# hmc-lair-shark-tracking/auv-sim

Hardware: AMD Instinct MI355X
Metric: RRT-Dubins node expansions/s (RRT.exploring) (higher is better)
Workload: dtype f64; 1 GPU; RRT.exploring 256 obst 200x200 cells 10000 iters x 12288 episodes/GPU, timebin parent sampling; episodes_per_gpu=12288, iters=10000, obstacles=256, cells=40000, parallelism=episodes sharded x1

## Files before the change

auv_sim_amd/_lib.py:

```python
import ctypes as C
import os

import numpy as np

HERE = os.path.dirname(os.path.abspath(__file__))
LIB_PATH = os.environ.get("AUVPLAN_LIBRARY") or os.path.join(HERE, "libauvplan.so")

_dp = C.POINTER(C.c_double)
_ip = C.POINTER(C.c_int32)
_bp = C.POINTER(C.c_int8)


class AuvpError(RuntimeError):
    def __init__(self, code, msg):
        super().__init__("auvplan error %d: %s" % (code, msg))
        self.code = code


class RRTParams(C.Structure):
    _fields_ = [("dist_to_end", C.c_double), ("diff_max", C.c_double), ("freq", C.c_double),
                ("min_dist", C.c_double), ("bin_interval", C.c_double), ("v", C.c_double),
                ("max_traj_time", C.c_double), ("max_plan_time", C.c_double), ("w", C.c_double * 3),
                ("mode", C.c_int32), ("max_iter", C.c_int32), ("points_per_iter", C.c_double)]

# ... 78 lines not shown
    L.auvp_math_dev.argtypes = [vp, C.c_int32, C.c_int32, _dp, _dp, _dp, _dp]
    L.auvp_nn_closest_batch.argtypes = [vp, C.c_int32, _dp, C.c_int32, _dp, C.c_int32, _ip, _ip]
    L.auvp_random_stream_dev.argtypes = [vp, C.c_uint64, C.c_int32, _dp]
    L.auvp_rrt_phase_clocks.argtypes = [vp, C.POINTER(C.c_uint64)]
    L.auvp_last_kernel_ms.argtypes = [vp]
    L.auvp_last_kernel_ms.restype = C.c_double
    L.auvp_last_launch.argtypes = [vp, _ip, _ip, _ip]
    L.auvp_rrt_last_launch_parts.argtypes = [vp, _dp, _dp, _ip]
    L.auvp_rrt_last_leaf_stats.argtypes = [vp, C.POINTER(C.c_int64)]
    L.auvp_rrt_last_kernel.argtypes = [vp]
    L.auvp_rrt_last_kernel.restype = C.c_char_p
    L.auvp_rrt_last_stream_ms.argtypes = [vp]
    L.auvp_rrt_last_stream_ms.restype = C.c_double
    L.auvp_rrt_last_stream_len.argtypes = [vp]
    L.auvp_rrt_last_stream_len.restype = C.c_int64
    L.auvp_hbm_probe.argtypes = [vp, C.c_uint64, C.c_int32, _dp, _dp]
    L.auvp_set_option.argtypes = [vp, C.c_char_p, C.c_int64]
    L.auvp_unset_option.argtypes = [vp, C.c_char_p]
    L.auvp_get_option.argtypes = [vp, C.c_char_p, _ip, C.POINTER(C.c_int64)]
    L.auvp_pipeline_fallbacks.argtypes = [vp, _ip, C.POINTER(C.c_int64)]
    _lib = L
    return L


OPTION_NAMES = ("ROWS", "DUO", "TRIO", "QUAD", "TIGHT_CULL", "NN_EXACT", "LEAF_SWEEP_ALL", "NO_HABITAT_GRID", "RG_MAX_ENTRIES",
                "NO_GRID_INDEX", "PRRT_LAT", "PRRT_PIPE", "PRRT_OBST_LDS", "PRRT_NEXT_LDS", "PRRT_ROWS", "ASTAR_NO_GRID",
                "ASTAR_NO_LIST", "ASTAR_PAIR", "SOG_TILE", "PIPE_FALLBACK", "PRRT_PIPE_DRAW", "PRRT_BUCKET_LDS", "ROWS_STREAM", "ROWS_STREAM_CAP", "ROWS_STREAM_WAVES",
                "ROWS_WG_WAVES")


def _f64(a, shape=None):
    a = np.ascontiguousarray(np.asarray(a, dtype=np.float64))
    return a.reshape(shape) if shape is not None else a


def _p(a, t=_dp):
    return a.ctypes.data_as(t)


def episode_limits(n_episodes, max_traj_time, habitat_keep, n_habitats, mode="timebin", iter_log=False, phase_clocks=False):
    E = int(n_episodes)
    if mode != "timebin":
        raise ValueError("per-episode limits need time-bin mode, not %r" % (mode,))
# ... 2 lines not shown
    mtt = np.broadcast_to(np.asarray(max_traj_time, dtype=np.float64), (E,))
    if not np.all(mtt > 0) or not np.all(np.isfinite(mtt)):
        raise ValueError("every max_traj_time must be finite and > 0")
    allowed = (1 << int(n_habitats)) - 1 if n_habitats < 64 else (1 << 64) - 1
    if habitat_keep is None:
        keep = [allowed] * E
    else:
        keep = [int(k) for k in np.broadcast_to(np.asarray(habitat_keep, dtype=object), (E,))]
    for e, k in enumerate(keep):
        if k < 0 or k & ~allowed:
            raise ValueError("episode %d: habitat_keep 0x%x names habitats outside the table of %d" % (e, k, n_habitats))
    rec = np.zeros(E, dtype=EPISODE_DTYPE)
    rec["max_traj_time"] = mtt
    rec["habitat_keep"] = np.array(keep, dtype=np.uint64)
    return float(mtt.max()), rec


class Context:

    def __init__(self, device=0):
        self.L = load()
        self.h = C.c_void_p()
        rc = self.L.auvp_create(int(device), C.byref(self.h))
        if rc != 0:
            raise AuvpError(rc, "auvp_create(device=%d) failed: no usable HIP device (no CPU fallback)" % device)
        self.device = int(device)
        self.n_episodes = 0
        self.max_iter = 0
        self.world_sizes = {}

# ... 198 lines not shown
        self.L.auvp_prrt_last_kernel.restype = C.c_char_p
        self.L.auvp_prrt_last_kernel.argtypes = [C.c_void_p]
        return (self.L.auvp_prrt_last_kernel(self.h) or b"").decode()

    def last_kernel_ms(self):
        return float(self.L.auvp_last_kernel_ms(self.h))

    def last_launch_parts(self):
        a, b, k = C.c_double(), C.c_double(), C.c_int32()
        self._chk(self.L.auvp_rrt_last_launch_parts(self.h, C.byref(a), C.byref(b), C.byref(k)))
        return a.value, b.value, k.value

    def last_stream_ms(self):
        return float(self.L.auvp_rrt_last_stream_ms(self.h))

    def last_stream_len(self):
        return int(self.L.auvp_rrt_last_stream_len(self.h))

    def last_rrt_kernel(self):
        return (self.L.auvp_rrt_last_kernel(self.h) or b"").decode()

    def last_leaf_stats(self):
        out = (C.c_int64 * 4)()
        self._chk(self.L.auvp_rrt_last_leaf_stats(self.h, out))
        return dict(zip(("nodes_visited", "points_visited", "elements_resummed", "leaves_resummed"), (int(v) for v in out)))

    def hbm_probe(self, n_bytes=4 << 30, reps=3):
        r, c = C.c_double(), C.c_double()
        self._chk(self.L.auvp_hbm_probe(self.h, int(n_bytes), int(reps), C.byref(r), C.byref(c)))
        return r.value, c.value
# ... 6 lines not shown
```

auv_sim_amd/csrc/auvplan.hip:

```cpp
#include <hip/hip_runtime.h>

#include <algorithm>
#include <cmath>
#include <cstdarg>
#include <cstdio>
#include <cstring>
#include <string>
#include <vector>

#include "../../include/auvplan.h"
#include "auvp_seed.h"
#include "rrt_explore_kernel.h"
#include "rrt_rows_kernel.h"
#include "rrt_rows_stream_kernel.h"
#include "rrt_duo_kernel.h"
#include "rrt_trio_kernel.h"

using namespace auvp;

extern "C" hipError_t auvpi_rrt_stream_launch(const auvp::RrtBuffers* B, int n_episodes, hipStream_t stream);
extern "C" hipError_t auvpi_rrt_rows_stream_launch(const auvp::WorldDev* W, const auvp::RrtParamsDev* P, const auvp::RrtBuffers* B, int n_episodes,
                                                   int grid, int block, int lds_max, int lds, hipStream_t stream);
extern "C" hipError_t auvpi_rrt_rows_launch(const auvp::WorldDev* W, const auvp::RrtParamsDev* P, const auvp::RrtBuffers* B, int n_episodes,
                                            int grid, int block, int lds_max, int lds, hipStream_t stream);

static_assert(sizeof(auvp_rrt_summary) == sizeof(RrtSummary), "summary layout");

namespace {

struct DevBuf {
  void* p = nullptr;
  size_t cap = 0;
  ~DevBuf() { if (p) (void)hipFree(p); }
  hipError_t reserve(size_t bytes) {
    if (bytes <= cap) return hipSuccess;
    release();
    hipError_t e = hipMalloc(&p, bytes ? bytes : 16);
    if (e == hipSuccess) cap = bytes ? bytes : 16;
    return e;
  }
  void release() { if (p) { (void)hipFree(p); p = nullptr; cap = 0; } }
  template <class T> T* as() const { return reinterpret_cast<T*>(p); }
};

}

enum AuvpOpt {
  OPT_ROWS, OPT_DUO, OPT_TRIO, OPT_QUAD, OPT_TIGHT_CULL, OPT_NN_EXACT, OPT_LEAF_SWEEP_ALL, OPT_NO_HABITAT_GRID, OPT_RG_MAX_ENTRIES,
  OPT_NO_GRID_INDEX, OPT_PRRT_LAT, OPT_PRRT_PIPE, OPT_PRRT_OBST_LDS, OPT_PRRT_NEXT_LDS, OPT_PRRT_ROWS, OPT_ASTAR_NO_GRID,
  OPT_ASTAR_NO_LIST, OPT_ASTAR_PAIR, OPT_SOG_TILE, OPT_PIPE_FALLBACK, OPT_PRRT_PIPE_DRAW, OPT_PRRT_BUCKET_LDS, OPT_ROWS_STREAM, OPT_ROWS_STREAM_CAP, OPT_ROWS_STREAM_WAVES, OPT_ROWS_WG_WAVES, OPT_COUNT
};
static const char* const AUVP_OPT_NAMES[OPT_COUNT] = {
  "ROWS", "DUO", "TRIO", "QUAD", "TIGHT_CULL", "NN_EXACT", "LEAF_SWEEP_ALL", "NO_HABITAT_GRID", "RG_MAX_ENTRIES",
  "NO_GRID_INDEX", "PRRT_LAT", "PRRT_PIPE", "PRRT_OBST_LDS", "PRRT_NEXT_LDS", "PRRT_ROWS", "ASTAR_NO_GRID",
  "ASTAR_NO_LIST", "ASTAR_PAIR", "SOG_TILE", "PIPE_FALLBACK", "PRRT_PIPE_DRAW", "PRRT_BUCKET_LDS", "ROWS_STREAM", "ROWS_STREAM_CAP", "ROWS_STREAM_WAVES", "ROWS_WG_WAVES"};

struct auvp_handle {
  bool opt_has[OPT_COUNT] = {};
  long long opt_val[OPT_COUNT] = {};
  bool opt_flag(int k, bool dflt) const { return opt_has[k] ? opt_val[k] != 0 : dflt; }
  bool opt_on(int k) const { return opt_has[k] && opt_val[k] != 0; }
  long long opt_num(int k, long long dflt) const { return opt_has[k] ? opt_val[k] : dflt; }
  int device = 0;
  hipStream_t stream = nullptr;
  hipEvent_t ev0 = nullptr, ev1 = nullptr, ev_mid = nullptr, ev_pre = nullptr;
  double last_expand_ms = 0.0, last_leaf_ms = 0.0, last_stream_ms = 0.0;
  long long last_stream_len = 0;
  struct Drawn { RrtParamsDev P{}; long long most = 0; int E = 0; unsigned long long used = 0; bool valid = false; };
  Drawn drawn[4];
  unsigned long long drawn_clock = 0;
  Drawn* drawn_find(const RrtParamsDev& P) {
    for (Drawn& d : drawn)
      if (d.valid && memcmp(&d.P, &P, sizeof P) == 0) return &d;
    return nullptr;
  }
  int last_rows = 0;
  const char* last_rrt_kernel = "";
  std::string err;
  bool have_world = false;
  double obst_area = 0.0;
  WorldDev W{};
  DevBuf d_ox, d_oy, d_ot, d_hab, d_habt, d_poly, d_bins, d_cells, d_prob, d_xoff, d_xitems, d_xdata, d_rgfirst, d_rgbp, d_rgoff,
// ... 763 lines not shown
    hipError_t e = hipFuncSetAttribute(reinterpret_cast<const void*>(kern), hipFuncAttributeMaxDynamicSharedMemorySize, (int)lds);
    if (e != hipSuccess) return e;
    hipLaunchKernelGGL(kern, dim3(grid), dim3(xw * 64), lds, h->stream, h->W, PR, B, (int)E, h->max_pts);
    return hipGetLastError();
  };
  if (B.leaf_stats) HIPCHK(h, hipMemsetAsync(B.leaf_stats, 0, 8 * sizeof(unsigned long long), h->stream));
  HIPCHK(h, hipEventRecord(h->ev0, h->stream));
  hipError_t le = hipSuccess;
  const RowsLdsPlan rp = rrt_rows_lds_plan(P.K, RW_MAX_OBST, rrt_tables_bytes(h->W.n_habitats, h->W.n_poly, h->W.n_bins));
  const bool iter_log = (P.flags & (AUVP_FLAG_ITER_LOG | AUVP_FLAG_PHASE_CLOCKS)) != 0;
  const bool rows_ok = !h->lim && P.mode == 0 && !iter_log && nfreq <= RW_MAX_FREQ && O_ <= RW_MAX_OBST && P.max_iter < 65534 &&
                       rp.total <= 160 * 1024;
  const bool use_rows = rows_ok && h->opt_flag(OPT_ROWS, E > 18 * n_cu_);
  int grid_used = grid, block_used = xw * 64, lds_used = (int)lds;
  bool stream_launched = false;
  const bool duo_ok = !h->lim && P.mode == 0 && !diag && nfreq <= DUO_MAX_FREQ && nfreq >= 1 && O_ <= 256 && h->max_pts <= 64;
  const bool use_duo = duo_ok && !use_rows && !one_wave_only && h->opt_flag(OPT_DUO, E <= 8 * n_cu_);
  const bool use_trio = duo_ok && !use_rows && !one_wave_only && h->opt_flag(OPT_TRIO, E <= TRIO_EP * n_cu_ && !h->opt_on(OPT_DUO));
  h->last_rrt_kernel = use_rows ? "rrt_rows_kernel" : (use_trio ? "rrt_trio_kernel" : (use_duo ? "rrt_duo_kernel" : "rrt_explore_kernel"));
  if (h->lim) h->last_rrt_kernel = "rrt_explore_lim_kernel";
  h->last_stream_ms = 0.0;
  h->last_stream_len = 0;
  if (use_trio) {
    int eps_wg = (E + n_cu_ - 1) / n_cu_;
    eps_wg = eps_wg < 1 ? 1 : (eps_wg > TRIO_EP ? TRIO_EP : eps_wg);
    const int jd = O_ <= 64 ? 1 : (O_ <= 128 ? 2 : 4);
    const int dl = trio_lds_bytes(P.K, jd * 64, rrt_tables_bytes(h->W.n_habitats, h->W.n_poly, h->W.n_bins), eps_wg);
    if (dl > 160 * 1024) return fail(h, AUVP_ERR_ARG, "LDS need %d B > 160 KiB (K=%d)", dl, P.K);
    const bool quad = h->opt_flag(OPT_QUAD, E <= n_cu_);
    grid_used = (E + eps_wg - 1) / eps_wg; block_used = eps_wg * (quad ? 256 : 192); lds_used = dl;
// ... 38 lines not shown
      cap = rrt_stream_len(h, seen);
      if (cap > 0x7fffffffll) use_stream = false;
      else if (!rrt_stream_reserve(h, (size_t)E * (size_t)cap * sizeof(double), &grew)) {
        if (h->opt_on(OPT_ROWS_STREAM)) return fail(h, AUVP_ERR_CAPACITY, "ROWS_STREAM = 1: %zu bytes of random stream do not fit the free memory", (size_t)E * (size_t)cap * sizeof(double));
        use_stream = false;
      }
    }
    if (grew) HIPCHK(h, hipEventRecord(h->ev0, h->stream));
    if (use_stream) {
      RrtBuffers Bs = B;
      Bs.stream = h->d_stream.as<double>();
      Bs.stream_cap = cap;
      int sw = (int)h->opt_num(OPT_ROWS_WG_WAVES, (E + RW_ROWS * n_cu - 1) / (RW_ROWS * n_cu));
      const int sw_max = (int)h->opt_num(OPT_ROWS_STREAM_WAVES, RW_WAVES);
      sw = sw < 1 ? 1 : (sw > sw_max ? sw_max : sw);
      sw = sw > RW_WAVES ? RW_WAVES : sw;
      while (sw > 1 && rrt_rows_stream_lds_plan(P.K, RW_MAX_OBST, rrt_tables_bytes(h->W.n_habitats, h->W.n_poly, h->W.n_bins), sw).total > 160 * 1024) sw--;
      const RowsStreamLdsPlan sp = rrt_rows_stream_lds_plan(P.K, RW_MAX_OBST, rrt_tables_bytes(h->W.n_habitats, h->W.n_poly, h->W.n_bins), sw);
      const RowsStreamLdsPlan sp_max = sp;
      grid_used = (E + sw * RW_ROWS - 1) / (sw * RW_ROWS); block_used = sw * 64;
      lds_used = sp.total;
      h->last_rrt_kernel = "rrt_rows_stream_kernel";
      h->last_stream_len = cap;
      le = auvpi_rrt_stream_launch(&Bs, (int)E, h->stream);
      if (le == hipSuccess) le = hipEventRecord(h->ev_pre, h->stream);
      if (le == hipSuccess) le = auvpi_rrt_rows_stream_launch(&h->W, &PR, &Bs, (int)E, grid_used, block_used, sp_max.total, sp.total, h->stream);
      stream_launched = true;
    } else
    le = auvpi_rrt_rows_launch(&h->W, &PR, &B, (int)E, grid_used, block_used, rp.total, rq.total, h->stream);
  } else {
  const int jsel = O <= 64 ? 0 : (O <= 128 ? 1 : (O <= 256 ? 2 : (O <= 512 ? 3 : 4)));
  const RrtEpisodeLimDev* lim = h->d_lim.as<RrtEpisodeLimDev>();
  auto launch_lim = [&](auto kern) -> hipError_t {
    hipError_t e = hipFuncSetAttribute(reinterpret_cast<const void*>(kern), hipFuncAttributeMaxDynamicSharedMemorySize, (int)lds);
    if (e != hipSuccess) return e;
    hipLaunchKernelGGL(kern, dim3(grid), dim3(xw * 64), lds, h->stream, h->W, PR, B, (int)E, h->max_pts, lim);
    return hipGetLastError();
  };
#define AUVP_LAUNCH_J(JV)                                                                   \
  do {                                                                                      \
    if (h->lim) le = launch_lim(rrt_explore_lim_kernel<JV>);                                \
// ... 226 lines not shown
double auvp_last_kernel_ms(auvp_handle* h) { return h ? h->last_ms : -1.0; }

int auvp_rrt_last_launch_parts(auvp_handle* h, double* expand_ms, double* leaf_ms, int32_t* episodes_per_wave) {
  if (!h) return AUVP_ERR_ARG;
  if (!h->have_batch) return fail(h, AUVP_ERR_STATE, "no batch has run");
  if (expand_ms) *expand_ms = h->last_expand_ms;
  if (leaf_ms) *leaf_ms = h->last_leaf_ms;
  if (episodes_per_wave) *episodes_per_wave = h->last_rows ? 4 : 1;
  return AUVP_OK;
}

const char* auvp_rrt_last_kernel(auvp_handle* h) { return h ? h->last_rrt_kernel : ""; }

double auvp_rrt_last_stream_ms(auvp_handle* h) { return h ? h->last_stream_ms : -1.0; }
int64_t auvp_rrt_last_stream_len(auvp_handle* h) { return h ? (int64_t)h->last_stream_len : -1; }

int auvp_rrt_last_leaf_stats(auvp_handle* h, int64_t* out4) {
  if (!h || !out4) return AUVP_ERR_ARG;
  if (!h->have_batch || !h->B.leaf_stats) return fail(h, AUVP_ERR_STATE, "no batch has run");
  HIPCHK(h, hipSetDevice(h->device));
  HIPCHK(h, hipMemcpy(out4, h->B.leaf_stats, 4 * sizeof(int64_t), hipMemcpyDeviceToHost));
  return AUVP_OK;
}

int auvp_last_launch(auvp_handle* h, int32_t* grid, int32_t* block, int32_t* lds_bytes) {
  if (!h) return AUVP_ERR_ARG;
  if (grid) *grid = h->last_grid;
  if (block) *block = h->last_block;
  if (lds_bytes) *lds_bytes = h->last_lds;
  return AUVP_OK;
// ... 29 lines not shown
```

auv_sim_amd/csrc/rows_kernels.hip:

```cpp
#include <hip/hip_runtime.h>
#include <stdint.h>

#include "rrt_rows_kernel.h"
#include "rrt_rows_stream_kernel.h"
#include "rrt_stream_kernel.h"

extern "C" __attribute__((visibility("hidden"))) hipError_t auvpi_rrt_rows_launch(const auvp::WorldDev* W, const auvp::RrtParamsDev* P,
                                                                                  const auvp::RrtBuffers* B, int n_episodes, int grid,
                                                                                  int block, int lds_max, int lds, hipStream_t stream) {
  hipError_t e = hipFuncSetAttribute(reinterpret_cast<const void*>(auvp::rrt_rows_kernel), hipFuncAttributeMaxDynamicSharedMemorySize, lds_max);
  if (e != hipSuccess) return e;
  hipLaunchKernelGGL(auvp::rrt_rows_kernel, dim3(grid), dim3(block), lds, stream, *W, *P, *B, n_episodes);
  return hipGetLastError();
}

extern "C" __attribute__((visibility("hidden"))) hipError_t auvpi_rrt_stream_launch(const auvp::RrtBuffers* B, int n_episodes, hipStream_t stream) {
  const int grid = (n_episodes + auvp::RSTREAM_WAVES - 1) / auvp::RSTREAM_WAVES;
  hipLaunchKernelGGL(auvp::rrt_stream_kernel, dim3(grid), dim3(auvp::RSTREAM_WAVES * 64), 0, stream, *B, n_episodes);
  return hipGetLastError();
}
extern "C" __attribute__((visibility("hidden"))) hipError_t auvpi_rrt_rows_stream_launch(const auvp::WorldDev* W, const auvp::RrtParamsDev* P,
                                                                                         const auvp::RrtBuffers* B, int n_episodes, int grid,
                                                                                         int block, int lds_max, int lds, hipStream_t stream) {
  auto go = [&](auto kern) -> hipError_t {
    hipError_t e = hipFuncSetAttribute(reinterpret_cast<const void*>(kern), hipFuncAttributeMaxDynamicSharedMemorySize, lds_max);
    if (e != hipSuccess) return e;
    hipLaunchKernelGGL(kern, dim3(grid), dim3(block), lds, stream, *W, *P, *B, n_episodes);
    return hipGetLastError();
  };
  return go(auvp::rrt_rows_stream_kernel<auvp::RW_WAVES>);
}
```

auv_sim_amd/csrc/rrt_rows_body.h:

```cpp
  extern __shared__ __align__(16) unsigned char smem[];
  const RrtTables S = rrt_tables_view(smem, W.n_habitats, W.n_poly);
  const int wave = (int)(threadIdx.x >> 6);
  const int lane = lane_id();
  const int row = lane >> 4, rl = lane & 15, rowbase = lane & 48;
  const int K = P.K;
  const int wg_waves = (int)(blockDim.x >> 6);
#if AUVP_ROWS_BODY_STREAM
  const RowsStreamLdsPlan plan = rrt_rows_stream_lds_plan(K, RW_MAX_OBST, rrt_tables_bytes(W.n_habitats, W.n_poly, W.n_bins), wg_waves);
  unsigned char* ebase = smem + plan.tables + (size_t)(wave * RW_ROWS + row) * plan.per_ep;
  double* ring = reinterpret_cast<double*>(ebase);
  double* inc = reinterpret_cast<double*>(ebase + plan.ring);
  uint16_t* bin_count = reinterpret_cast<uint16_t*>(ebase + plan.ring + plan.scratch);
#else
  const RowsLdsPlan plan = rrt_rows_lds_plan(K, RW_MAX_OBST, rrt_tables_bytes(W.n_habitats, W.n_poly, W.n_bins), wg_waves);
  unsigned char* ebase = smem + plan.tables + (size_t)(wave * RW_ROWS + row) * plan.per_ep;
  uint32_t* mt = reinterpret_cast<uint32_t*>(ebase);
  double* win = reinterpret_cast<double*>(ebase + plan.mt);
  double* inc = win;
  uint16_t* bin_count = reinterpret_cast<uint16_t*>(ebase + plan.mt + plan.scratch);
#endif

  rrt_tables_stage(S, W);
  if (threadIdx.x == 0) *S.params = P;
  const RrtParamsDev& Q = *S.params;
// ... 12 lines not shown
  double* nodeF = B.node_f + (size_t)eps * capn * 8;
  int4* nodeI = reinterpret_cast<int4*>(B.node_i) + (size_t)eps * capn;
  uint8_t* nodeQ = B.node_q + (size_t)eps * capn;
  double* ptF = B.points + (size_t)eps * capp * 6;
  const BinLists bins = bin_lists(B, (size_t)eps, K);
  int next_chunk = 0;
  const double* init = B.init + (size_t)eps * 6;

#if AUVP_ROWS_BODY_STREAM
  RowStream rng;
  rng.ring = ring;
  rng.src = B.stream + (size_t)eps * (size_t)B.stream_cap;
  rng.pos = 0u; rng.front = 0u; rng.req = 0u;
  rng.cap = (uint32_t)B.stream_cap;
#pragma unroll
  for (int c = 0; c < RS_PEND; c++) rng.pend[c] = 0.0;
#define ROWS_CONSUME(on, n) stream_advance(rng, on, (uint32_t)(n))
#else
  RowRng rng;
  rng.s = mt;
  for (int i = rl; i < 624; i += 16) mt[i] = B.mt[(size_t)eps * 624 + i];
  {
    int idx = B.mt_index ? B.mt_index[eps] : 624;
    idx = idx < 0 ? 0 : (idx > 624 ? 624 : idx);
    rng.pslot = idx == 624 ? 0u : (uint32_t)idx;
    rng.avail = (uint32_t)(624 - idx);
    rng.drawn = 0ull;
  }
#define ROWS_CONSUME(on, n) rows_advance(rng, on, (uint32_t)(2 * (n)))
#endif
  for (int i = rl; i < K + 2; i += 16) bin_count[i] = 0;
// ... 5 lines not shown
    bins.direct[(K >= 1 ? 1 : 0) * AUVP_BIN_HEAD] = 0;
    bin_count[K >= 1 ? 1 : 0] = 1;
  }
  wave_sync();
  int n_nodes = 1, n_points = 0, status = 0, n_cand = 0, iters_run = 0;
  const double4 sbox = reinterpret_cast<const double4*>(W.os_box)[rl];
  const int nv_poly = W.n_poly;

  for (int it = 0; it < P.max_iter; it++) {
    if (!wave_any(live)) break;
    int par = 0, n_total = 0, base = 0;
    {
      bool search = live;
      int fo = 0, rb = 0, cnt = 0;
      double u = 0.0;
      for (;;) {
#if AUVP_ROWS_BODY_STREAM
        if (!stream_ensure(rng, search, 16u, rl) && search) { status = AUVP_ST_STREAM; live = false; iters_run = it; search = false; }
        if (search) u = stream_at(rng, (uint32_t)rl);
#else
        rows_ensure(rng, search, 32u, rl);
        if (search) { u = rows_random_at(rng, (uint32_t)rl); win[rl] = u; }
#endif
        const int rbj = (int)py_uniform(1.0, (double)(K + 1), u);
        const bool cand = search && rl < 14;
        const bool badkey = cand && rbj > K;
        const int cj = (cand && !badkey) ? (int)bin_count[rbj] : 0;
        const uint32_t okm = row_ballot(cj != 0, rowbase), badm = row_ballot(badkey, rowbase);
        const int f_ok = okm ? (__ffs((int)okm) - 1) : 16, f_bad = badm ? (__ffs((int)badm) - 1) : 16;
        if (search) {
          if (f_bad < f_ok) { status = -5; live = false; iters_run = it; search = false; }
          else if (f_ok < 16) { fo = f_ok; search = false; }
        }
        const bool again = search;
        ROWS_CONSUME(again, 14);
        const int src = rowbase + (again ? 0 : fo);
        const int rb_n = row_read(rbj, src), cnt_n = row_read(cj, src);
        if (!again && live && cnt == 0) { rb = rb_n; cnt = cnt_n; }
        if (!wave_any(again)) break;
      }
#if AUVP_ROWS_BODY_STREAM
      const double u1 = stream_at(rng, (uint32_t)(fo + 1)), u2 = stream_at(rng, (uint32_t)(fo + 2));
#else
      wave_sync();
      const double u1 = win[fo + 1], u2 = win[fo + 2];
#endif
      if (live) {
        const int ri = (int)py_uniform(0.0, (double)cnt, u1);
        par = bin_member(bins, rb, ri);
        n_total = (int)auvp_floor(py_uniform(0.0, Q.freq, u2) / 1);
        base = fo + 3;
      }
    }
    const bool on0 = live && 0 < n_total;
    const int n0_ = on0 ? (n_total < RW_C ? n_total : RW_C) : 0;
#if AUVP_ROWS_BODY_STREAM
    if (!stream_ensure(rng, on0, (uint32_t)(base + 3 * n0_), rl) && on0) { status = AUVP_ST_STREAM; live = false; iters_run = it; }
#else
    auto make_window = [&](bool on, int nwin, int b0) {
      rows_ensure(rng, on, (uint32_t)(2 * (b0 + nwin)), rl);
#pragma unroll
      for (int t = 0; t < 3; t++) {
        const int j = rl + 16 * t;
        if (on && j < nwin) win[j] = rows_random_at(rng, (uint32_t)(b0 + j));
      }
      wave_sync();
    };
    {
      const int e_end = base + 3 * n0_;
      rows_ensure(rng, on0, (uint32_t)(2 * e_end), rl);
#pragma unroll
      for (int t = 0; t < 3; t++) {
        const int e = 16 + rl + 16 * t;
        if (on0 && e < e_end) win[e] = rows_random_at(rng, (uint32_t)e);
      }
      wave_sync();
    }
#endif
    double cx = 0.0, cy = 0.0, cth = 0.0, ctt = 0.0, clen = 0.0;
    if (live) {
      const double2 a = *reinterpret_cast<const double2*>(nodeF + (size_t)par * 8);
      const double2 b = *reinterpret_cast<const double2*>(nodeF + (size_t)par * 8 + 2);
      cx = a.x; cy = a.y; cth = b.x; ctt = b.y;
      clen = nodeF[(size_t)par * 8 + 4];
    }
#if AUVP_ROWS_BODY_STREAM
    stream_top_up(rng, live, rl);
#endif
    const double px0 = cx, py0 = cy, clen0 = clen;
    int cnt = 0;
    double ptx[2] = {0.0, 0.0}, pty[2] = {0.0, 0.0};
    bool ptv[2] = {false, false};
    bool first_pass = true;
#pragma unroll
    for (int pass = 0; pass < 2; pass++) {
      const int c0 = pass * RW_C;
      const bool on = live && c0 < n_total;
      if (!wave_any(on)) break;
      const int n = on ? ((n_total - c0) < RW_C ? (n_total - c0) : RW_C) : 0;
      const int nwin = 3 * n;
#ifdef AUVP_ROWS_PAD
      {
        double pd0 = cth, pd1 = cx, pd2 = cy, pd3 = ctt;
#pragma unroll
        for (int q = 0; q < AUVP_ROWS_PAD / 4; q++)
          asm volatile("v_add_f64 %0, %0, 1.0\n\tv_add_f64 %1, %1, 1.0\n\tv_add_f64 %2, %2, 1.0\n\tv_add_f64 %3, %3, 1.0"
                       : "+v"(pd0), "+v"(pd1), "+v"(pd2), "+v"(pd3));
      }
#endif
      const int b0 = first_pass ? base : 0;
#if AUVP_ROWS_BODY_STREAM
      if (pass != 0 && !stream_ensure(rng, on, (uint32_t)nwin, rl) && on) { status = AUVP_ST_STREAM; live = false; iters_run = it; }
      const uint32_t wb = (uint32_t)b0;
#define ROWS_WIN(j) stream_at(rng, wb + (uint32_t)(j))
#else
      if (pass != 0) make_window(on, nwin, b0);
      const double* wp = win + (pass == 0 ? base : 0);
#define ROWS_WIN(j) wp[j]
#endif
      unsigned long long tpred = 0ull;
#pragma unroll
      for (int t = 0; t < 3; t++) {
        const int j = rl + 16 * t;
        const double dist = py_uniform(0.0, Q.dist_to_end, ROWS_WIN(j));
        const double diff = py_uniform(-Q.diff_max, Q.diff_max, ROWS_WIN(j + 1));
        const unsigned long long fb = __builtin_amdgcn_fcmp(auvp_fabs(dist), auvp_fabs(diff), 2 ) &
                                      __builtin_amdgcn_uicmp((unsigned)(j + 1), (unsigned)nwin, 36 );
        tpred |= ((fb >> rowbase) & 0xffffull) << (16 * t);
      }
// ... 198 lines not shown
          nf[4] = clen;
          nodeI[me] = make_int4(it, par, n_points, cnt);
          nodeQ[me] = ctt >= Q.max_traj_time - 30 ? 1 : 0;
        }
        n_nodes++;
        n_points += cnt;
      }
    }
    wave_sync();
  }

  const bool valid = ep < n_episodes;
  if (live) iters_run = P.max_iter;
#if AUVP_ROWS_BODY_STREAM
  const unsigned long long drawn = 2ull * rng.pos;
  if (!stream_ensure(rng, valid && status == 0, 1u, rl) && valid && status == 0) status = AUVP_ST_STREAM;
  const double after = status == AUVP_ST_STREAM ? 0.0 : stream_at(rng, 0u);
#else
  const unsigned long long drawn = rng.drawn;
  rows_ensure(rng, valid, 2u, rl);
  const double after = rows_random_at(rng, 0u);
#endif
  if (valid) {
    for (int i = rl; i < K + 1; i += 16) B.bin_count[(size_t)ep * (K + 1) + i] = (int32_t)bin_count[i];
    if (rl == 0) {
      RrtSummary& s = B.summary[ep];
#if AUVP_ROWS_BODY_STREAM
      pipe_report(B.pipe_fail, status == AUVP_ST_STREAM ? AUVP_ST_PIPELINE : 0);
#endif
      s.status = status; s.n_nodes = n_nodes; s.n_points = n_points; s.n_leaves = 0;
      s.best_leaf = -1; s.best_path_len = 0; s.iters_run = iters_run; s.n_candidates = n_cand;
      s.best_cost[0] = __builtin_inf(); s.best_cost[1] = 0.0; s.best_cost[2] = 0.0; s.best_cost[3] = 0.0;
      s.best_length = 0.0;
      s.rng_after = after; s.leaf_elems = 0; s.n_draw32 = drawn; s.nn_scanned = 0ull;
    }
  }
#undef ROWS_CONSUME
```

auv_sim_amd/csrc/rrt_rows_stream_kernel.h:

```cpp
#ifndef AUVP_RRT_ROWS_STREAM_KERNEL_H
#define AUVP_RRT_ROWS_STREAM_KERNEL_H
#include "rrt_rows_kernel.h"

namespace auvp {

constexpr int RS_RING = 256;
constexpr int RS_WAVES = 16;
constexpr int RS_PEND = 4;

struct RowsStreamLdsPlan {
  int tables, ring, scratch, bins, per_ep, obst, total;
};
__host__ __device__ inline RowsStreamLdsPlan rrt_rows_stream_lds_plan(int K, int n_obst_slots, int tables_bytes, int waves = RW_WAVES) {
  RowsStreamLdsPlan p;
  p.tables = (tables_bytes + 15) & ~15;
  p.ring = RS_RING * 8;
  p.scratch = (4 * 18 * 8 + 15) & ~15;
  p.bins = (((K + 2) * 2) + 15) & ~15;
  p.per_ep = p.ring + p.scratch + p.bins;
  p.obst = n_obst_slots * (8 + 8 + 4);
  p.total = p.tables + waves * RW_ROWS * p.per_ep + p.obst;
  return p;
}

struct RowStream {
  double* ring;
  const double* src;
  uint32_t pos, front, req, cap;
  double pend[RS_PEND];
};

__device__ __forceinline__ void stream_commit(RowStream& r, int rl) {
#pragma unroll
  for (int c = 0; c < RS_PEND; c++)
    if (r.front + 16u * (uint32_t)c < r.req) r.ring[(r.front + 16u * (uint32_t)c + (uint32_t)rl) & (uint32_t)(RS_RING - 1)] = r.pend[c];
  r.front = r.req;
}
__device__ __forceinline__ void stream_request(RowStream& r, bool on, int rl) {
  const uint32_t room = (uint32_t)RS_RING - (r.front - r.pos);
  uint32_t n = room >> 4;
  n = n > (uint32_t)RS_PEND ? (uint32_t)RS_PEND : n;
  n = on ? n : 0u;
#pragma unroll
  for (int c = 0; c < RS_PEND; c++) {
    const uint32_t e = r.req + 16u * (uint32_t)c + (uint32_t)rl;
    if ((uint32_t)c < n && e < r.cap) r.pend[c] = __builtin_nontemporal_load(r.src + e);
  }
  r.req += 16u * n;
}
__device__ __forceinline__ void stream_top_up(RowStream& r, bool on, int rl) {
  stream_commit(r, rl);
  stream_request(r, on, rl);
}
__device__ __forceinline__ bool stream_ensure(RowStream& r, bool want, uint32_t need, int rl) {
  const uint32_t need_w = want ? need : 0u;
  const bool ok = r.pos + need_w <= r.cap;
  for (;;) {
    if (__builtin_amdgcn_uicmp(r.front - r.pos, ok ? need_w : 0u, 36 ) == 0ull) break;
    const bool go = ok && r.front - r.pos < need_w;
    stream_commit(r, rl);
    stream_request(r, go && ok, rl);
    stream_commit(r, rl);
    wave_sync();
    if (!wave_any(go && ok && r.front - r.pos < need_w)) break;
  }
  wave_sync();
  return ok;
}
__device__ __forceinline__ double stream_at(const RowStream& r, uint32_t j) { return r.ring[(r.pos + j) & (uint32_t)(RS_RING - 1)]; }
__device__ __forceinline__ void stream_advance(RowStream& r, bool on, uint32_t n) {
  if (on) r.pos += n;
}

template <int MAXW>
static __global__ __launch_bounds__(MAXW * 64, 1) void rrt_rows_stream_kernel(WorldDev W, RrtParamsDev P, RrtBuffers B, int n_episodes) {
#define AUVP_ROWS_BODY_STREAM 1
#include "rrt_rows_body.h"
#undef AUVP_ROWS_BODY_STREAM
}

}
#endif
```

include/auvplan.h:

```cpp
#ifndef AUVPLAN_H
#define AUVPLAN_H
#include <stdint.h>

#ifdef __cplusplus
extern "C" {
#endif

typedef struct auvp_handle auvp_handle;

enum {
  AUVP_OK = 0,
  AUVP_NO_QUALIFYING_LEAF = 1,
  AUVP_ERR_ARG = -1,
  AUVP_ERR_CAPACITY = -2,
  AUVP_ERR_HIP = -3,
  AUVP_ERR_STATE = -4,
  AUVP_ERR_KEY = -5,
  AUVP_ERR_COMM = -6,
  AUVP_ERR_GENERATOR = -7,
  AUVP_ERR_PIPELINE = -9
  ,
  AUVP_ERR_STREAM = -10
};

// ... 167 lines not shown
int auvp_cost_paths(auvp_handle* h, int32_t n_paths, const int32_t* off, const double* pts_xyt,
                    const int32_t* bin_lo, const int32_t* bin_hi, const double* total_traj_time,
                    const double* weights3, double* out4);
int auvp_nn_closest_batch(auvp_handle* h, int32_t n_nodes, const double* xy, int32_t n_queries, const double* q,
                          int32_t force_exact, int32_t* out_index, int32_t* out_slow);
int auvp_hbm_probe(auvp_handle* h, uint64_t bytes, int32_t reps, double* read_GBps, double* copy_GBps);
int auvp_sincos_dev(auvp_handle* h, int32_t n, const double* x, double* s, double* c);
int auvp_math_dev(auvp_handle* h, int32_t op, int32_t n, const double* a, const double* b, double* out0, double* out1);
int auvp_random_stream_dev(auvp_handle* h, uint64_t seed, int32_t n, double* out);

int auvp_rrt_phase_clocks(auvp_handle* h, uint64_t* out);
double auvp_last_kernel_ms(auvp_handle* h);
int auvp_rrt_last_launch_parts(auvp_handle* h, double* expand_ms, double* leaf_ms, int32_t* episodes_per_wave);
double auvp_rrt_last_stream_ms(auvp_handle* h);
int64_t auvp_rrt_last_stream_len(auvp_handle* h);
const char* auvp_rrt_last_kernel(auvp_handle* h);
int auvp_rrt_last_leaf_stats(auvp_handle* h, int64_t* out4);
int auvp_last_launch(auvp_handle* h, int32_t* grid, int32_t* block, int32_t* lds_bytes);

int auvp_prrt_replan_particles(auvp_handle* h, const double* start4, const auvp_prrt_params* params, const double* xform,
                               const double* clamp4, uint64_t seed_base, int32_t flags);

#define AUVP_COMM_ID_BYTES 128
int auvp_comm_unique_id(uint8_t* id_out );
int auvp_comm_init(auvp_handle* h, int32_t world_size, int32_t rank, const uint8_t* id);
int auvp_comm_destroy(auvp_handle* h);
int auvp_gather(auvp_handle* h, const void* send_dev, size_t bytes_per_rank, void* recv_dev);
int auvp_gather_var(auvp_handle* h, const void* send_dev, int64_t send_bytes, void* recv_dev, int64_t recv_cap_bytes,
                    int64_t* counts_out);
int auvp_gather_counts(auvp_handle* h, int64_t send_bytes, int64_t* counts_out );
// ... 17 lines not shown
```

Before: 1.262 billion expansions/s.

## Add mirrored LDS ring tail and vectorized f64x2 stream loads for rows-stream RRT

The random-number ring in LDS gains a mirrored tail of 48 extra slots, so window reads can use a plain base-plus-offset address without masking on every access. Global stream loads and LDS commits now move two doubles per lane as an f64x2 vector, with fewer pending chunks. A shape planner picks waves per workgroup and whether the mirror fits the LDS budget, and can drop waves to make it fit. The costs are extra LDS per episode, which may reduce waves per workgroup, and a new requirement that the stream capacity is a multiple of 64.

```diff
diff --git a/auv_sim_amd/_lib.py b/auv_sim_amd/_lib.py
--- a/auv_sim_amd/_lib.py
+++ b/auv_sim_amd/_lib.py
@@ -116,6 +116,9 @@
     L.auvp_rrt_last_stream_ms.restype = C.c_double
     L.auvp_rrt_last_stream_len.argtypes = [vp]
     L.auvp_rrt_last_stream_len.restype = C.c_int64
+    if hasattr(L, "auvp_rrt_last_stream_mirror"):
+        L.auvp_rrt_last_stream_mirror.argtypes = [vp]
+        L.auvp_rrt_rows_stream_shape.argtypes = [C.c_int32] * 6 + [_ip, _ip, _ip]
     L.auvp_hbm_probe.argtypes = [vp, C.c_uint64, C.c_int32, _dp, _dp]
     L.auvp_set_option.argtypes = [vp, C.c_char_p, C.c_int64]
     L.auvp_unset_option.argtypes = [vp, C.c_char_p]
@@ -128,7 +131,7 @@
 OPTION_NAMES = ("ROWS", "DUO", "TRIO", "QUAD", "TIGHT_CULL", "NN_EXACT", "LEAF_SWEEP_ALL", "NO_HABITAT_GRID", "RG_MAX_ENTRIES",
                 "NO_GRID_INDEX", "PRRT_LAT", "PRRT_PIPE", "PRRT_OBST_LDS", "PRRT_NEXT_LDS", "PRRT_ROWS", "ASTAR_NO_GRID",
                 "ASTAR_NO_LIST", "ASTAR_PAIR", "SOG_TILE", "PIPE_FALLBACK", "PRRT_PIPE_DRAW", "PRRT_BUCKET_LDS", "ROWS_STREAM", "ROWS_STREAM_CAP", "ROWS_STREAM_WAVES",
-                "ROWS_WG_WAVES")
+                "ROWS_WG_WAVES", "ROWS_STREAM_MIRROR")
 
 
 def _f64(a, shape=None):
@@ -161,6 +164,15 @@
     rec["max_traj_time"] = mtt
     rec["habitat_keep"] = np.array(keep, dtype=np.uint64)
     return float(mtt.max()), rec
+
+
+def rows_stream_shape(K, n_habitats, n_poly, n_bins, waves_wanted=12, force=-1):
+    w, m, l = C.c_int32(), C.c_int32(), C.c_int32()
+    rc = load().auvp_rrt_rows_stream_shape(int(K), int(n_habitats), int(n_poly), int(n_bins), int(waves_wanted), int(force),
+                                           C.byref(w), C.byref(m), C.byref(l))
+    if rc != 0:
+        raise AuvpError(rc, "auvp_rrt_rows_stream_shape: bad argument")
+    return w.value, bool(m.value), l.value
 
 
 class Context:
@@ -389,6 +401,9 @@
     def last_stream_ms(self):
         return float(self.L.auvp_rrt_last_stream_ms(self.h))
 
+    def last_stream_mirror(self):
+        return int(self.L.auvp_rrt_last_stream_mirror(self.h))
+
     def last_stream_len(self):
         return int(self.L.auvp_rrt_last_stream_len(self.h))
 
diff --git a/auv_sim_amd/csrc/auvplan.hip b/auv_sim_amd/csrc/auvplan.hip
--- a/auv_sim_amd/csrc/auvplan.hip
+++ b/auv_sim_amd/csrc/auvplan.hip
@@ -20,7 +20,7 @@
 
 extern "C" hipError_t auvpi_rrt_stream_launch(const auvp::RrtBuffers* B, int n_episodes, hipStream_t stream);
 extern "C" hipError_t auvpi_rrt_rows_stream_launch(const auvp::WorldDev* W, const auvp::RrtParamsDev* P, const auvp::RrtBuffers* B, int n_episodes,
-                                                   int grid, int block, int lds_max, int lds, hipStream_t stream);
+                                                   int grid, int block, int lds_max, int lds, int mirror, hipStream_t stream);
 extern "C" hipError_t auvpi_rrt_rows_launch(const auvp::WorldDev* W, const auvp::RrtParamsDev* P, const auvp::RrtBuffers* B, int n_episodes,
                                             int grid, int block, int lds_max, int lds, hipStream_t stream);
 
@@ -48,12 +48,12 @@
 enum AuvpOpt {
   OPT_ROWS, OPT_DUO, OPT_TRIO, OPT_QUAD, OPT_TIGHT_CULL, OPT_NN_EXACT, OPT_LEAF_SWEEP_ALL, OPT_NO_HABITAT_GRID, OPT_RG_MAX_ENTRIES,
   OPT_NO_GRID_INDEX, OPT_PRRT_LAT, OPT_PRRT_PIPE, OPT_PRRT_OBST_LDS, OPT_PRRT_NEXT_LDS, OPT_PRRT_ROWS, OPT_ASTAR_NO_GRID,
-  OPT_ASTAR_NO_LIST, OPT_ASTAR_PAIR, OPT_SOG_TILE, OPT_PIPE_FALLBACK, OPT_PRRT_PIPE_DRAW, OPT_PRRT_BUCKET_LDS, OPT_ROWS_STREAM, OPT_ROWS_STREAM_CAP, OPT_ROWS_STREAM_WAVES, OPT_ROWS_WG_WAVES, OPT_COUNT
+  OPT_ASTAR_NO_LIST, OPT_ASTAR_PAIR, OPT_SOG_TILE, OPT_PIPE_FALLBACK, OPT_PRRT_PIPE_DRAW, OPT_PRRT_BUCKET_LDS, OPT_ROWS_STREAM, OPT_ROWS_STREAM_CAP, OPT_ROWS_STREAM_WAVES, OPT_ROWS_WG_WAVES, OPT_ROWS_STREAM_MIRROR, OPT_COUNT
 };
 static const char* const AUVP_OPT_NAMES[OPT_COUNT] = {
   "ROWS", "DUO", "TRIO", "QUAD", "TIGHT_CULL", "NN_EXACT", "LEAF_SWEEP_ALL", "NO_HABITAT_GRID", "RG_MAX_ENTRIES",
   "NO_GRID_INDEX", "PRRT_LAT", "PRRT_PIPE", "PRRT_OBST_LDS", "PRRT_NEXT_LDS", "PRRT_ROWS", "ASTAR_NO_GRID",
-  "ASTAR_NO_LIST", "ASTAR_PAIR", "SOG_TILE", "PIPE_FALLBACK", "PRRT_PIPE_DRAW", "PRRT_BUCKET_LDS", "ROWS_STREAM", "ROWS_STREAM_CAP", "ROWS_STREAM_WAVES", "ROWS_WG_WAVES"};
+  "ASTAR_NO_LIST", "ASTAR_PAIR", "SOG_TILE", "PIPE_FALLBACK", "PRRT_PIPE_DRAW", "PRRT_BUCKET_LDS", "ROWS_STREAM", "ROWS_STREAM_CAP", "ROWS_STREAM_WAVES", "ROWS_WG_WAVES", "ROWS_STREAM_MIRROR"};
 
 struct auvp_handle {
   bool opt_has[OPT_COUNT] = {};
@@ -66,6 +66,7 @@
   hipEvent_t ev0 = nullptr, ev1 = nullptr, ev_mid = nullptr, ev_pre = nullptr;
   double last_expand_ms = 0.0, last_leaf_ms = 0.0, last_stream_ms = 0.0;
   long long last_stream_len = 0;
+  int last_stream_mirror = -1;
   struct Drawn { RrtParamsDev P{}; long long most = 0; int E = 0; unsigned long long used = 0; bool valid = false; };
   Drawn drawn[4];
   unsigned long long drawn_clock = 0;
@@ -859,6 +860,7 @@
   const bool use_rows = rows_ok && h->opt_flag(OPT_ROWS, E > 18 * n_cu_);
   int grid_used = grid, block_used = xw * 64, lds_used = (int)lds;
   bool stream_launched = false;
+  h->last_stream_mirror = -1;
   const bool duo_ok = !h->lim && P.mode == 0 && !diag && nfreq <= DUO_MAX_FREQ && nfreq >= 1 && O_ <= 256 && h->max_pts <= 64;
   const bool use_duo = duo_ok && !use_rows && !one_wave_only && h->opt_flag(OPT_DUO, E <= 8 * n_cu_);
   const bool use_trio = duo_ok && !use_rows && !one_wave_only && h->opt_flag(OPT_TRIO, E <= TRIO_EP * n_cu_ && !h->opt_on(OPT_DUO));
@@ -927,17 +929,19 @@
       int sw = (int)h->opt_num(OPT_ROWS_WG_WAVES, (E + RW_ROWS * n_cu - 1) / (RW_ROWS * n_cu));
       const int sw_max = (int)h->opt_num(OPT_ROWS_STREAM_WAVES, RW_WAVES);
       sw = sw < 1 ? 1 : (sw > sw_max ? sw_max : sw);
-      sw = sw > RW_WAVES ? RW_WAVES : sw;
-      while (sw > 1 && rrt_rows_stream_lds_plan(P.K, RW_MAX_OBST, rrt_tables_bytes(h->W.n_habitats, h->W.n_poly, h->W.n_bins), sw).total > 160 * 1024) sw--;
-      const RowsStreamLdsPlan sp = rrt_rows_stream_lds_plan(P.K, RW_MAX_OBST, rrt_tables_bytes(h->W.n_habitats, h->W.n_poly, h->W.n_bins), sw);
+      const RowsStreamShape shape = rrt_rows_stream_shape(P.K, RW_MAX_OBST, rrt_tables_bytes(h->W.n_habitats, h->W.n_poly, h->W.n_bins), sw,
+                                                          h->opt_has[OPT_ROWS_STREAM_MIRROR] ? (h->opt_val[OPT_ROWS_STREAM_MIRROR] != 0 ? 1 : 0) : -1);
+      sw = shape.waves;
+      const RowsStreamLdsPlan sp = shape.plan;
       const RowsStreamLdsPlan sp_max = sp;
+      h->last_stream_mirror = shape.mirror ? 1 : 0;
       grid_used = (E + sw * RW_ROWS - 1) / (sw * RW_ROWS); block_used = sw * 64;
       lds_used = sp.total;
       h->last_rrt_kernel = "rrt_rows_stream_kernel";
       h->last_stream_len = cap;
       le = auvpi_rrt_stream_launch(&Bs, (int)E, h->stream);
       if (le == hipSuccess) le = hipEventRecord(h->ev_pre, h->stream);
-      if (le == hipSuccess) le = auvpi_rrt_rows_stream_launch(&h->W, &PR, &Bs, (int)E, grid_used, block_used, sp_max.total, sp.total, h->stream);
+      if (le == hipSuccess) le = auvpi_rrt_rows_stream_launch(&h->W, &PR, &Bs, (int)E, grid_used, block_used, sp_max.total, sp.total, shape.mirror ? 1 : 0, h->stream);
       stream_launched = true;
     } else
     le = auvpi_rrt_rows_launch(&h->W, &PR, &B, (int)E, grid_used, block_used, rp.total, rq.total, h->stream);
@@ -1194,6 +1198,17 @@
 
 double auvp_rrt_last_stream_ms(auvp_handle* h) { return h ? h->last_stream_ms : -1.0; }
 int64_t auvp_rrt_last_stream_len(auvp_handle* h) { return h ? (int64_t)h->last_stream_len : -1; }
+int auvp_rrt_last_stream_mirror(auvp_handle* h) { return h ? h->last_stream_mirror : -1; }
+
+int auvp_rrt_rows_stream_shape(int32_t K, int32_t n_habitats, int32_t n_poly, int32_t n_bins, int32_t waves_wanted, int32_t force,
+                               int32_t* waves, int32_t* mirror, int32_t* lds_bytes) {
+  if (K < 0 || n_habitats < 0 || n_poly < 0 || n_bins < 0) return AUVP_ERR_ARG;
+  const RowsStreamShape s = rrt_rows_stream_shape(K, RW_MAX_OBST, rrt_tables_bytes(n_habitats, n_poly, n_bins), waves_wanted, force);
+  if (waves) *waves = s.waves;
+  if (mirror) *mirror = s.mirror ? 1 : 0;
+  if (lds_bytes) *lds_bytes = s.plan.total;
+  return AUVP_OK;
+}
 
 int auvp_rrt_last_leaf_stats(auvp_handle* h, int64_t* out4) {
   if (!h || !out4) return AUVP_ERR_ARG;
diff --git a/auv_sim_amd/csrc/rows_kernels.hip b/auv_sim_amd/csrc/rows_kernels.hip
--- a/auv_sim_amd/csrc/rows_kernels.hip
+++ b/auv_sim_amd/csrc/rows_kernels.hip
@@ -21,12 +21,13 @@
 }
 extern "C" __attribute__((visibility("hidden"))) hipError_t auvpi_rrt_rows_stream_launch(const auvp::WorldDev* W, const auvp::RrtParamsDev* P,
                                                                                          const auvp::RrtBuffers* B, int n_episodes, int grid,
-                                                                                         int block, int lds_max, int lds, hipStream_t stream) {
+                                                                                         int block, int lds_max, int lds, int mirror, hipStream_t stream) {
+  if (B->stream_cap <= 0 || B->stream_cap % 64 != 0) return hipErrorInvalidValue;
   auto go = [&](auto kern) -> hipError_t {
     hipError_t e = hipFuncSetAttribute(reinterpret_cast<const void*>(kern), hipFuncAttributeMaxDynamicSharedMemorySize, lds_max);
     if (e != hipSuccess) return e;
     hipLaunchKernelGGL(kern, dim3(grid), dim3(block), lds, stream, *W, *P, *B, n_episodes);
     return hipGetLastError();
   };
-  return go(auvp::rrt_rows_stream_kernel<auvp::RW_WAVES>);
+  return mirror ? go(auvp::rrt_rows_stream_kernel<auvp::RW_WAVES>) : go(auvp::rrt_rows_stream_masked_kernel<auvp::RW_WAVES>);
 }
diff --git a/auv_sim_amd/csrc/rrt_rows_body.h b/auv_sim_amd/csrc/rrt_rows_body.h
--- a/auv_sim_amd/csrc/rrt_rows_body.h
+++ b/auv_sim_amd/csrc/rrt_rows_body.h
@@ -6,7 +6,7 @@
   const int K = P.K;
   const int wg_waves = (int)(blockDim.x >> 6);
 #if AUVP_ROWS_BODY_STREAM
-  const RowsStreamLdsPlan plan = rrt_rows_stream_lds_plan(K, RW_MAX_OBST, rrt_tables_bytes(W.n_habitats, W.n_poly, W.n_bins), wg_waves);
+  const RowsStreamLdsPlan plan = rrt_rows_stream_lds_plan(K, RW_MAX_OBST, rrt_tables_bytes(W.n_habitats, W.n_poly, W.n_bins), wg_waves, MIRROR);
   unsigned char* ebase = smem + plan.tables + (size_t)(wave * RW_ROWS + row) * plan.per_ep;
   double* ring = reinterpret_cast<double*>(ebase);
   double* inc = reinterpret_cast<double*>(ebase + plan.ring);
@@ -50,7 +50,10 @@
   rng.pos = 0u; rng.front = 0u; rng.req = 0u;
   rng.cap = (uint32_t)B.stream_cap;
 #pragma unroll
-  for (int c = 0; c < RS_PEND; c++) rng.pend[c] = 0.0;
+  for (int c = 0; c < RS_PEND; c++) rng.pend[c] = rs_piece(0.0);
+#ifdef AUVP_STREAM_COUNT_SLOW
+  rng.slow = 0u;
+#endif
 #define ROWS_CONSUME(on, n) stream_advance(rng, on, (uint32_t)(n))
 #else
   RowRng rng;
@@ -86,10 +89,14 @@
       bool search = live;
       int fo = 0, rb = 0, cnt = 0;
       double u = 0.0;
+#if AUVP_ROWS_BODY_STREAM
+      StreamBase<MIRROR> sel;
+#endif
       for (;;) {
 #if AUVP_ROWS_BODY_STREAM
-        if (!stream_ensure(rng, search, 16u, rl) && search) { status = AUVP_ST_STREAM; live = false; iters_run = it; search = false; }
-        if (search) u = stream_at(rng, (uint32_t)rl);
+        if (!stream_ensure<MIRROR>(rng, search, 16u, rl) && search) { status = AUVP_ST_STREAM; live = false; iters_run = it; search = false; }
+        sel = stream_base<MIRROR>(rng, 0u, rl);
+        if (search) u = stream_read(sel, rl, rl);
 #else
         rows_ensure(rng, search, 32u, rl);
         if (search) { u = rows_random_at(rng, (uint32_t)rl); win[rl] = u; }
@@ -112,7 +119,7 @@
         if (!wave_any(again)) break;
       }
 #if AUVP_ROWS_BODY_STREAM
-      const double u1 = stream_at(rng, (uint32_t)(fo + 1)), u2 = stream_at(rng, (uint32_t)(fo + 2));
+      const double u1 = stream_read(sel, fo + 1, rl), u2 = stream_read(sel, fo + 2, rl);
 #else
       wave_sync();
       const double u1 = win[fo + 1], u2 = win[fo + 2];
@@ -127,7 +134,7 @@
     const bool on0 = live && 0 < n_total;
     const int n0_ = on0 ? (n_total < RW_C ? n_total : RW_C) : 0;
 #if AUVP_ROWS_BODY_STREAM
-    if (!stream_ensure(rng, on0, (uint32_t)(base + 3 * n0_), rl) && on0) { status = AUVP_ST_STREAM; live = false; iters_run = it; }
+    if (!stream_ensure<MIRROR>(rng, on0, (uint32_t)(base + 3 * n0_), rl) && on0) { status = AUVP_ST_STREAM; live = false; iters_run = it; }
 #else
     auto make_window = [&](bool on, int nwin, int b0) {
       rows_ensure(rng, on, (uint32_t)(2 * (b0 + nwin)), rl);
@@ -157,7 +164,7 @@
       clen = nodeF[(size_t)par * 8 + 4];
     }
 #if AUVP_ROWS_BODY_STREAM
-    stream_top_up(rng, live, rl);
+    stream_top_up<MIRROR>(rng, live, rl);
 #endif
     const double px0 = cx, py0 = cy, clen0 = clen;
     int cnt = 0;
@@ -182,9 +189,9 @@
 #endif
       const int b0 = first_pass ? base : 0;
 #if AUVP_ROWS_BODY_STREAM
-      if (pass != 0 && !stream_ensure(rng, on, (uint32_t)nwin, rl) && on) { status = AUVP_ST_STREAM; live = false; iters_run = it; }
-      const uint32_t wb = (uint32_t)b0;
-#define ROWS_WIN(j) stream_at(rng, wb + (uint32_t)(j))
+      if (pass != 0 && !stream_ensure<MIRROR>(rng, on, (uint32_t)nwin, rl) && on) { status = AUVP_ST_STREAM; live = false; iters_run = it; }
+      const StreamBase<MIRROR> wb = stream_base<MIRROR>(rng, (uint32_t)b0, rl);
+#define ROWS_WIN(j) stream_read(wb, (j), rl)
 #else
       if (pass != 0) make_window(on, nwin, b0);
       const double* wp = win + (pass == 0 ? base : 0);
@@ -413,8 +420,8 @@
   if (live) iters_run = P.max_iter;
 #if AUVP_ROWS_BODY_STREAM
   const unsigned long long drawn = 2ull * rng.pos;
-  if (!stream_ensure(rng, valid && status == 0, 1u, rl) && valid && status == 0) status = AUVP_ST_STREAM;
-  const double after = status == AUVP_ST_STREAM ? 0.0 : stream_at(rng, 0u);
+  if (!stream_ensure<MIRROR>(rng, valid && status == 0, 1u, rl) && valid && status == 0) status = AUVP_ST_STREAM;
+  const double after = status == AUVP_ST_STREAM ? 0.0 : stream_read(stream_base<MIRROR>(rng, 0u, rl), rl, rl);
 #else
   const unsigned long long drawn = rng.drawn;
   rows_ensure(rng, valid, 2u, rl);
@@ -432,6 +439,9 @@
       s.best_cost[0] = __builtin_inf(); s.best_cost[1] = 0.0; s.best_cost[2] = 0.0; s.best_cost[3] = 0.0;
       s.best_length = 0.0;
       s.rng_after = after; s.leaf_elems = 0; s.n_draw32 = drawn; s.nn_scanned = 0ull;
+#if AUVP_ROWS_BODY_STREAM && defined(AUVP_STREAM_COUNT_SLOW)
+      s.nn_scanned = rng.slow;
+#endif
     }
   }
 #undef ROWS_CONSUME
diff --git a/auv_sim_amd/csrc/rrt_rows_stream_kernel.h b/auv_sim_amd/csrc/rrt_rows_stream_kernel.h
--- a/auv_sim_amd/csrc/rrt_rows_stream_kernel.h
+++ b/auv_sim_amd/csrc/rrt_rows_stream_kernel.h
@@ -5,16 +5,27 @@
 namespace auvp {
 
 constexpr int RS_RING = 256;
+constexpr int RS_MIRROR = 48;
 constexpr int RS_WAVES = 16;
-constexpr int RS_PEND = 4;
+#ifndef AUVP_RS_PIECE
+#define AUVP_RS_PIECE 2
+#endif
+constexpr int RS_PIECE = AUVP_RS_PIECE;
+constexpr int RS_CHUNK = 16 * RS_PIECE;
+constexpr int RS_PEND = 64 / RS_CHUNK;
+typedef double rs_f64x2 __attribute__((ext_vector_type(2)));
+template <int N> struct RsPiece { typedef double type; };
+template <> struct RsPiece<2> { typedef rs_f64x2 type; };
+typedef RsPiece<RS_PIECE>::type rs_piece;
+constexpr int RS_LDS_LIMIT = 160 * 1024;
 
 struct RowsStreamLdsPlan {
   int tables, ring, scratch, bins, per_ep, obst, total;
 };
-__host__ __device__ inline RowsStreamLdsPlan rrt_rows_stream_lds_plan(int K, int n_obst_slots, int tables_bytes, int waves = RW_WAVES) {
+__host__ __device__ inline RowsStreamLdsPlan rrt_rows_stream_lds_plan(int K, int n_obst_slots, int tables_bytes, int waves = RW_WAVES, bool mirror = false) {
   RowsStreamLdsPlan p;
   p.tables = (tables_bytes + 15) & ~15;
-  p.ring = RS_RING * 8;
+  p.ring = (RS_RING + (mirror ? RS_MIRROR : 0)) * 8;
   p.scratch = (4 * 18 * 8 + 15) & ~15;
   p.bins = (((K + 2) * 2) + 15) & ~15;
   p.per_ep = p.ring + p.scratch + p.bins;
@@ -23,57 +34,102 @@
   return p;
 }
 
+struct RowsStreamShape {
+  int waves;
+  bool mirror;
+  RowsStreamLdsPlan plan;
+};
+__host__ inline RowsStreamShape rrt_rows_stream_shape(int K, int n_obst_slots, int tables_bytes, int waves_wanted, int force = -1) {
+  int sw = waves_wanted < 1 ? 1 : (waves_wanted > RW_WAVES ? RW_WAVES : waves_wanted);
+  while (sw > 1 && rrt_rows_stream_lds_plan(K, n_obst_slots, tables_bytes, sw, false).total > RS_LDS_LIMIT) sw--;
+  bool mirror = force < 0 ? rrt_rows_stream_lds_plan(K, n_obst_slots, tables_bytes, sw, true).total <= RS_LDS_LIMIT : force != 0;
+  while (mirror && sw > 1 && rrt_rows_stream_lds_plan(K, n_obst_slots, tables_bytes, sw, true).total > RS_LDS_LIMIT) sw--;
+  RowsStreamShape s;
+  s.waves = sw; s.mirror = mirror;
+  s.plan = rrt_rows_stream_lds_plan(K, n_obst_slots, tables_bytes, sw, mirror);
+  return s;
+}
+
 struct RowStream {
   double* ring;
   const double* src;
   uint32_t pos, front, req, cap;
-  double pend[RS_PEND];
+  rs_piece pend[RS_PEND];
+#ifdef AUVP_STREAM_COUNT_SLOW
+  uint32_t slow;
+#endif
 };
 
+template <bool MIRROR>
 __device__ __forceinline__ void stream_commit(RowStream& r, int rl) {
 #pragma unroll
   for (int c = 0; c < RS_PEND; c++)
-    if (r.front + 16u * (uint32_t)c < r.req) r.ring[(r.front + 16u * (uint32_t)c + (uint32_t)rl) & (uint32_t)(RS_RING - 1)] = r.pend[c];
+    if (r.front + (uint32_t)(RS_CHUNK * c) < r.req) {
+      const uint32_t s = (r.front + (uint32_t)(RS_CHUNK * c) + (uint32_t)(RS_PIECE * rl)) & (uint32_t)(RS_RING - 1);
+      *reinterpret_cast<rs_piece*>(r.ring + s) = r.pend[c];
+      if (MIRROR && s < (uint32_t)RS_MIRROR) *reinterpret_cast<rs_piece*>(r.ring + s + (uint32_t)RS_RING) = r.pend[c];
+    }
   r.front = r.req;
 }
 __device__ __forceinline__ void stream_request(RowStream& r, bool on, int rl) {
-  const uint32_t room = (uint32_t)RS_RING - (r.front - r.pos);
-  uint32_t n = room >> 4;
+  const uint32_t room = (uint32_t)RS_RING - (r.front - r.pos), left = r.cap - r.req;
+  uint32_t n = (room < left ? room : left) / (uint32_t)RS_CHUNK;
   n = n > (uint32_t)RS_PEND ? (uint32_t)RS_PEND : n;
   n = on ? n : 0u;
 #pragma unroll
-  for (int c = 0; c < RS_PEND; c++) {
-    const uint32_t e = r.req + 16u * (uint32_t)c + (uint32_t)rl;
-    if ((uint32_t)c < n && e < r.cap) r.pend[c] = __builtin_nontemporal_load(r.src + e);
-  }
-  r.req += 16u * n;
+  for (int c = 0; c < RS_PEND; c++)
+    if ((uint32_t)c < n)
+      r.pend[c] = __builtin_nontemporal_load(reinterpret_cast<const rs_piece*>(r.src + r.req + (uint32_t)(RS_CHUNK * c) + (uint32_t)(RS_PIECE * rl)));
+  r.req += (uint32_t)RS_CHUNK * n;
 }
+template <bool MIRROR>
 __device__ __forceinline__ void stream_top_up(RowStream& r, bool on, int rl) {
-  stream_commit(r, rl);
+  stream_commit<MIRROR>(r, rl);
   stream_request(r, on, rl);
 }
+template <bool MIRROR>
 __device__ __forceinline__ bool stream_ensure(RowStream& r, bool want, uint32_t need, int rl) {
   const uint32_t need_w = want ? need : 0u;
   const bool ok = r.pos + need_w <= r.cap;
   for (;;) {
     if (__builtin_amdgcn_uicmp(r.front - r.pos, ok ? need_w : 0u, 36 ) == 0ull) break;
     const bool go = ok && r.front - r.pos < need_w;
-    stream_commit(r, rl);
+#ifdef AUVP_STREAM_COUNT_SLOW
+    if (go) r.slow++;
+#endif
+    stream_commit<MIRROR>(r, rl);
     stream_request(r, go && ok, rl);
-    stream_commit(r, rl);
+    stream_commit<MIRROR>(r, rl);
     wave_sync();
     if (!wave_any(go && ok && r.front - r.pos < need_w)) break;
   }
   wave_sync();
   return ok;
 }
-__device__ __forceinline__ double stream_at(const RowStream& r, uint32_t j) { return r.ring[(r.pos + j) & (uint32_t)(RS_RING - 1)]; }
+template <bool MIRROR> struct StreamBase;
+template <> struct StreamBase<true> { const double* p; };
+template <> struct StreamBase<false> { const double* ring; uint32_t first; };
+template <bool MIRROR>
+__device__ __forceinline__ StreamBase<MIRROR> stream_base(const RowStream& r, uint32_t b, int rl) {
+  if constexpr (MIRROR) return StreamBase<true>{r.ring + (((r.pos + b) & (uint32_t)(RS_RING - 1)) + (uint32_t)rl)};
+  else return StreamBase<false>{r.ring, r.pos + b};
+}
+__device__ __forceinline__ double stream_read(const StreamBase<true>& w, int j, int rl) { return w.p[j - rl]; }
+__device__ __forceinline__ double stream_read(const StreamBase<false>& w, int j, int) { return w.ring[(w.first + (uint32_t)j) & (uint32_t)(RS_RING - 1)]; }
 __device__ __forceinline__ void stream_advance(RowStream& r, bool on, uint32_t n) {
   if (on) r.pos += n;
 }
 
 template <int MAXW>
 static __global__ __launch_bounds__(MAXW * 64, 1) void rrt_rows_stream_kernel(WorldDev W, RrtParamsDev P, RrtBuffers B, int n_episodes) {
+  constexpr bool MIRROR = true;
+#define AUVP_ROWS_BODY_STREAM 1
+#include "rrt_rows_body.h"
+#undef AUVP_ROWS_BODY_STREAM
+}
+template <int MAXW>
+static __global__ __launch_bounds__(MAXW * 64, 1) void rrt_rows_stream_masked_kernel(WorldDev W, RrtParamsDev P, RrtBuffers B, int n_episodes) {
+  constexpr bool MIRROR = false;
 #define AUVP_ROWS_BODY_STREAM 1
 #include "rrt_rows_body.h"
 #undef AUVP_ROWS_BODY_STREAM
diff --git a/include/auvplan.h b/include/auvplan.h
--- a/include/auvplan.h
+++ b/include/auvplan.h
@@ -205,6 +205,9 @@
 int auvp_rrt_last_launch_parts(auvp_handle* h, double* expand_ms, double* leaf_ms, int32_t* episodes_per_wave);
 double auvp_rrt_last_stream_ms(auvp_handle* h);
 int64_t auvp_rrt_last_stream_len(auvp_handle* h);
+int auvp_rrt_last_stream_mirror(auvp_handle* h);
+int auvp_rrt_rows_stream_shape(int32_t K, int32_t n_habitats, int32_t n_poly, int32_t n_bins, int32_t waves_wanted, int32_t force,
+                               int32_t* waves, int32_t* mirror, int32_t* lds_bytes);
 const char* auvp_rrt_last_kernel(auvp_handle* h);
 int auvp_rrt_last_leaf_stats(auvp_handle* h, int64_t* out4);
 int auvp_last_launch(auvp_handle* h, int32_t* grid, int32_t* block, int32_t* lds_bytes);
```

New measurement: 1.283 billion expansions/s, median of 6. 1.02x the previous value.
